# FrozenBurning/SceneDreamer

Hardware: AMD Instinct MI355X
Metric: rendered frames/sec @960×540, 24 samples/ray, scene_size 2048; HBM GB/s (higher is better)
Workload: dtype f16 (3-term split MFMA, f32 accumulate; f32 hash grid); 1 GPU; 960x540, num_samples=24, scene_size=2048, cam pattern 0 (pose stride 2 of 40 poses), 1 frame per rank per step; apron=minimal, parallelism=frames x1

## Files before the change

### scenedreamer_amd/csrc/field.hip

```cpp
#include <hip/hip_fp16.h>

#include <cstdlib>
#include <utility>

#include "field_composite.h"
#include "mlp_layers.h"
#include "sdn_common.h"

namespace {

typedef int i32x4v __attribute__((ext_vector_type(4)));

struct MlpParams {
    const float *feat;
    const float *dist;
    const uint8_t *label;
    const uint8_t *rayflag;
    const half8 *wpk;
    const float *consts;
    const float *sky_c;
    float *net_out;
    int32_t R, ns, nch, n_tiles;
    float term_depth;
    uint8_t *passes;
// ... 109 lines not shown
    const float *u;
    float *rand_depth;
    float *new_dists;
    int64_t *idx;
    int32_t R, M, n_points;
    int32_t ieee_div;
    float sample_depth;
};

__global__ __launch_bounds__(256) void sample_depth_kernel(const SampleParams p) {
    const int ray = blockIdx.x * 256 + threadIdx.x;
    if (ray >= p.R) return;
    RayBoxes rb;
#pragma unroll
    for (int k = 0; k < MAXM; k++) {
        if (k < p.M) {
            rb.t[k] = p.depth2[(size_t)ray * p.M + k];
            rb.t2[k] = p.depth2[((size_t)p.R + ray) * p.M + k];
        } else {
            rb.t[k] = rb.t2[k] = __builtin_nanf("");
        }
        rb.id[k] = 0;
    }
    const float *u = p.u ? p.u + (size_t)ray * p.n_points : nullptr;
    const int ns = p.n_points - 1;
    for (int i = 0; i < ns; i++) {
        Placed pl = place_sample(rb, p.M, p.lin, u, p.ieee_div ? -p.n_points : p.n_points, i, p.sample_depth);
        p.new_dists[(size_t)ray * ns + i] = pl.dist;
        p.rand_depth[(size_t)ray * ns + i] = pl.raw_depth;
        p.idx[(size_t)ray * ns + i] = pl.raw_idx;
    }
}

__device__ __forceinline__ void input_encode(const EncParams &enc, int rr, int rl, int sidx, bool ray_ok, bool use_feat, int h, half8 (&bh)[16],
                                             half8 (&bl)[16], int &lab, float &dist, bool &gnd, float &depth) {
    RayBoxes rb;
    float dd[3];
    enc_load_ray(enc, rr, rb, dd);
    const EncSample es = enc_place(enc, rb, dd, rl, sidx, ray_ok);
    gnd = gnd || es.gnd;
    lab = es.label;
    dist = es.dist;
    depth = es.depth;
#pragma unroll
    for (int b = 0; b < 2; b++) {
        float res[4][8];
        enc_levels<4>(enc, es, 4 * b, h, use_feat, res);
#pragma unroll
        for (int t = 0; t < 4; t++) split8(res[t], bh[4 * b + t], bl[4 * b + t]);
    }
}

template <int DBG>
__device__ __forceinline__ void input_buffer(const MlpParams &p, size_t tc, bool prefetched, bool tile_ok, int lane, int j, half8 (&bh)[16],
                                             half8 (&bl)[16], int &lab, float &dist) {
    float raw[8][8];
    if (prefetched) {
        if constexpr (DBG & 1) asm volatile("s_waitcnt vmcnt(0)" ::: "memory");
        else asm volatile("s_waitcnt vmcnt(16)" ::: "memory");
#define SDN_PF_READ8(S, A0, A1, A2, A3, A4, A5, A6, A7) \
    asm volatile("v_accvgpr_read_b32 %0, a" #A0 "\n\tv_accvgpr_read_b32 %1, a" #A1 "\n\tv_accvgpr_read_b32 %2, a" #A2 \
                 "\n\tv_accvgpr_read_b32 %3, a" #A3 "\n\tv_accvgpr_read_b32 %4, a" #A4 "\n\tv_accvgpr_read_b32 %5, a" #A5 \
                 "\n\tv_accvgpr_read_b32 %6, a" #A6 "\n\tv_accvgpr_read_b32 %7, a" #A7 \
                 : "=v"(raw[S][0]), "=v"(raw[S][1]), "=v"(raw[S][2]), "=v"(raw[S][3]), "=v"(raw[S][4]), "=v"(raw[S][5]), \
                   "=v"(raw[S][6]), "=v"(raw[S][7]))
        SDN_PF_READ8(0, 190, 191, 192, 193, 194, 195, 196, 197);
        SDN_PF_READ8(1, 198, 199, 200, 201, 202, 203, 204, 205);
        SDN_PF_READ8(2, 206, 207, 208, 209, 210, 211, 212, 213);
        SDN_PF_READ8(3, 214, 215, 216, 217, 218, 219, 220, 221);
        SDN_PF_READ8(4, 222, 223, 224, 225, 226, 227, 228, 229);
        SDN_PF_READ8(5, 230, 231, 232, 233, 234, 235, 236, 237);
        SDN_PF_READ8(6, 238, 239, 240, 241, 242, 243, 244, 245);
// ... 41 lines not shown
    asm volatile("global_load_dwordx4 a[" #R0 ":" #R0 "+3], %0, off\n\tglobal_load_dwordx4 a[" #R1 ":" #R1 "+3], %0, off offset:16\n\t" \
                 "global_load_dwordx4 a[" #R2 ":" #R2 "+3], %0, off offset:2048\n\tglobal_load_dwordx4 a[" #R3 ":" #R3 "+3], %0, off offset:2064" \
                 ::"v"(base + (K) * 4096) : "memory", SDN_PF_CLOBBERS)
#define SDN_PF_CLOBBERS "a190", "a191", "a192", "a193", "a194", "a195", "a196", "a197", "a198", "a199", "a200", "a201", "a202", "a203", "a204", "a205", "a206", "a207", "a208", "a209", "a210", "a211", "a212", "a213", "a214", "a215", "a216", "a217", "a218", "a219", "a220", "a221", "a222", "a223", "a224", "a225", "a226", "a227", "a228", "a229", "a230", "a231", "a232", "a233", "a234", "a235", "a236", "a237", "a238", "a239", "a240", "a241", "a242", "a243", "a244", "a245", "a246", "a247", "a248", "a249", "a250", "a251", "a252", "a253"
    SDN_PF_LOAD4(0, 190, 194, 198, 202);
    SDN_PF_LOAD4(1, 206, 210, 214, 218);
    SDN_PF_LOAD4(2, 222, 226, 230, 234);
    SDN_PF_LOAD4(3, 238, 242, 246, 250);
#undef SDN_PF_CLOBBERS
#undef SDN_PF_LOAD4
    asm volatile("global_load_ubyte a254, %0, off" ::"v"(p.label + (size_t)tn * 32 + j) : "memory", "a254");
    asm volatile("global_load_dword a255, %0, off" ::"v"(p.dist + (size_t)tn * 32 + j) : "memory", "a255");
}

__device__ __forceinline__ void flag_put(unsigned flags_a, int word, int v) {
    asm volatile("ds_write_b32 %0, %1" ::"v"(flags_a + 4u * (unsigned)word), "v"(v) : "memory");
}
__device__ __forceinline__ i32x4v flag_get4(unsigned flags_a, int word0) {
    i32x4v f;
    asm volatile("ds_read_b128 %0, %1\n\ts_waitcnt lgkmcnt(0)" : "=v"(f) : "v"(flags_a + 4u * (unsigned)word0) : "memory");
    return f;
}
__device__ __forceinline__ i32x4v workgroup_vote(unsigned flags_a, int word0, int lane, int wave, int mine) {
    if (lane == 0) flag_put(flags_a, word0 + wave, mine);
    asm volatile("s_waitcnt lgkmcnt(0)" ::: "memory");
    __builtin_amdgcn_s_barrier();
    return flag_get4(flags_a, word0);
}

template <int DBG, int CT, int MODE = MODE_BUFFER>
__global__ __launch_bounds__(256, 1) void mlp_kernel(const MlpParams p) {
    constexpr bool FUSED = MODE == MODE_FUSED || MODE == MODE_FUSED_AUX, AUX = MODE == MODE_FUSED_AUX, RAW = MODE == MODE_RAW;
    constexpr bool SKIP = MODE == MODE_FUSED;
    __shared__ __attribute__((aligned(1024))) char lds[LDS_TOTAL];
    const int lane = threadIdx.x & 63, wave = threadIdx.x >> 6;
    const int h = lane >> 5, j = lane & 31;
    const int q = j & 3;

    float *cst = reinterpret_cast<float *>(lds + LDS_CONST);
    stage_consts(cst, p.consts, p.sky_avg);
    EncParams enc = p.enc;
    if constexpr (FUSED)
        stage_enc_tables(enc, p.enc, reinterpret_cast<float *>(lds + LDS_ENC_SCALES), reinterpret_cast<float *>(lds + LDS_ENC_LIN),
                         reinterpret_cast<uint8_t *>(lds + LDS_ENC_LUT), p.cam_ori_dev);
    __syncthreads();

    Ring r;
    r.slots_per_pass = SLOTS_PER_PASS;
    r.wbytes = reinterpret_cast<const char *>(p.wpk);
    r.g = 0;
    r.wave = __builtin_amdgcn_readfirstlane(wave);
    r.lane = lane;
    r.voff = r.wave * (PIECES * 1024) + lane * 16;
    r.lds_lane = (unsigned)(size_t)(const lds_char *)(lds + LDS_RING) + lane * 16;
    r.src_delta = r.wave * (PIECES * 1024) - (int)(unsigned)(size_t)(const lds_char *)(lds + LDS_RING);
#pragma unroll
    for (int sl = 0; sl < DMA_AHEAD; sl++) ring_issue(lds, r, sl, sl);
    r.next_in_pass = DMA_AHEAD;

    unsigned t_seg = 0;
    if constexpr (DBG & 512) {
        if (threadIdx.x < 16) reinterpret_cast<unsigned *>(lds + LDS_TIMERS)[threadIdx.x] = 0u;
        t_seg = (unsigned)__builtin_readcyclecounter();
    }
    long pf_tc = -1;
    unsigned long long t_stage = 0, t_kernel0 = 0;
    unsigned n_pass = 0;
    if constexpr (DBG & 128) t_kernel0 = __builtin_readcyclecounter();
    const int n_groups = (p.n_tiles + 3) >> 2;
    const unsigned flags_a = lds_addr(lds + LDS_FLAGS);
    int grp = blockIdx.x, grp_next = blockIdx.x + (int)gridDim.x;
    auto first_vox = [&](int g) -> int {
        const int t = g * 4 + wave, ry = t * RAYS_PER_TILE + (j >> 2);
        if (!(g < n_groups && t < p.n_tiles && ry < p.R && enc.win.valid(ry))) return 0;
        return enc.voxel_id[(size_t)enc.win.src(ry) * enc.M];
    };
    int vox_cur = 0;
    if constexpr (FUSED) vox_cur = first_vox(grp);
    int cold = 0;
    while (grp < n_groups) {
        const int tile = grp * 4 + wave;
        const bool tile_ok = tile < p.n_tiles;
        const int tile_s = grp * 4 + r.wave;
        const bool tile_ok_s = tile_s < p.n_tiles;
        const int ray = tile * RAYS_PER_TILE + (j >> 2);
        const bool ray_ok = tile_ok && ray < p.R && (!FUSED || p.win.valid(ray));
        const int rl = ray_ok ? ray : p.R - 1;
        const int rr = FUSED ? enc.win.src(rl) : 0;
        uint8_t flag;
        int vox_nxt = 0;
        if constexpr (FUSED) {
            flag = vox_cur != 0 ? (uint8_t)0 : (uint8_t)1;
            vox_nxt = first_vox(grp_next);
        } else if constexpr (RAW) flag = tile_ok ? (uint8_t)0 : (uint8_t)1;
        else flag = ray_ok ? p.rayflag[ray] : (uint8_t)1;
        bool gnd = false;
        int drawn = grp_next + (int)gridDim.x;
        if (p.ticket && threadIdx.x == 0) drawn = 2 * (int)gridDim.x + atomicAdd(p.ticket, 1);
        const bool any_hit = AUX ? tile_ok : __any(!(flag & 1));
        if (threadIdx.x == 0) flag_put(flags_a, 4, drawn);
        const i32x4v fh = workgroup_vote(flags_a, 0, lane, wave, any_hit ? 1 : 0), fd = flag_get4(flags_a, 4);
        const bool grp_hit = __builtin_amdgcn_readfirstlane(fh[0] | fh[1] | fh[2] | fh[3]) != 0;
        const int grp_next2 = __builtin_amdgcn_readfirstlane(fd[0]);
        asm volatile("s_waitcnt lgkmcnt(0)" ::: "memory");
        __builtin_amdgcn_s_barrier();

        float outq[2][4] = {{0.f, 0.f, 0.f, 0.f}, {0.f, 0.f, 0.f, 0.f}};
        float carry = 0.f, tsum = 0.f;
        int n_done = 0, n_colour = 0;
        bool skip_test = SKIP && !p.no_colour_skip && (cold < 6 || (cold & 3) == 0);
        if (SKIP && !skip_test) cold++;

        for (int ch = 0; grp_hit && ch < p.nch; ch++) {
            const size_t tc = (size_t)(tile_ok ? tile : 0) * p.nch + ch;
            half8 bh[16], bl[16];
            f32x16 acc[8];
            MxState mx;
            if constexpr (CT == 6) {
#pragma unroll
                for (int k = 0; k < 4; k++) mx.bm[k] = 0.f;
            }
            seg_tick<DBG>(lds, 9, t_seg);
            unsigned long long t_in0 = 0;
            if constexpr (DBG & 128) t_in0 = __builtin_readcyclecounter();
            const long tc_s = (long)(tile_ok_s ? tile_s : 0) * p.nch + ch;
            int lab;
            float dist;
            float smp_depth = 0.f;
            const long row = (long)(tile_ok ? tile : 0) * 256 + ch * 32 + j;
            if constexpr (RAW) {
                const long rc = row < p.R ? row : (long)p.R - 1;
                lab = p.label[rc];
                dist = 0.f;
                const float *src = p.feat + rc * FEAT + 8 * h;
#pragma unroll
                for (int s = 0; s < 8; s++) {
                    const float4 a = *reinterpret_cast<const float4 *>(src + 16 * s), b = *reinterpret_cast<const float4 *>(src + 16 * s + 4);
                    const float v[8] = {a.x, a.y, a.z, a.w, b.x, b.y, b.z, b.w};
                    split8(v, bh[s], bl[s]);
                }
            }
            else if constexpr (FUSED)
                input_encode(enc, rr, rl, ch * SAMP_PER_STEP + (j & 3), ray_ok, AUX ? ray_ok : !(flag & 1), h, bh, bl, lab, dist, gnd, smp_depth);
            else input_buffer<DBG>(p, tc, pf_tc == tc_s && !(DBG & 256), tile_ok, lane, j, bh, bl, lab, dist);
            if constexpr (DBG & 128) {
                asm volatile("s_waitcnt vmcnt(0)" ::"v"(bh[7]), "v"(bl[7]) : "memory");
                t_stage += __builtin_readcyclecounter() - t_in0;
                n_pass++;
            }
            if constexpr (DBG & 512) asm volatile("s_waitcnt vmcnt(0)" ::"v"(bh[7]), "v"(bl[7]) : "memory");
            seg_tick<DBG>(lds, 0, t_seg);
            float part = 0.f;
            bool colour_skipped = false;
            const float *wsig = cst + C_WSIGMA;
            const float *bias1 = cst + C_LABEL_BIAS + lab * HID;
            layer8<DBG, 8, false, false, false>(lds, r, bh, bl, acc, bias1, bias1, wsig, h, part, TRUNK_K, TRUNK_K);
            act_step<7, false>(acc, bias1, wsig, h, bh, bl, part, TRUNK_K);
            seg_tick<DBG>(lds, 1, t_seg);
#pragma unroll 1
            for (int l = 0; l < 5; l++) {
                const float *bias = cst + C_BETA + l * HID;
                const float *bias_pend = l == 0 ? bias1 : bias - HID;
                constexpr float tk = TRUNK_K;
                if constexpr (CT == 6) {
                    if (l == 2) layer8x<DBG, 0, false, true>(lds, r, bh, bl, mx, acc, bias, bias_pend, wsig, h, part, tk, tk);
                    else if (l == 3) layer8x<DBG, 1, true, false>(lds, r, bh, bl, mx, acc, bias, bias_pend, wsig, h, part, 1.f, tk);
                    else if (l == 4) layer8x<DBG, 2, false, false>(lds, r, bh, bl, mx, acc, bias, bias_pend, wsig, h, part, 1.f, 1.f);
                    else layer8<DBG, 16, true, false, false>(lds, r, bh, bl, acc, bias, bias_pend, wsig, h, part, tk, tk);
                } else {
                    if (l == 2) layer8<DBG, 16, true, false, true, 3, true, CT == 3>(lds, r, bh, bl, acc, bias, bias_pend, wsig, h, part, tk, tk);
                    else if (l == 3) layer8<DBG, 16, true, true, false, CT, CT == 3, CT == 3>(lds, r, bh, bl, acc, bias, bias_pend, wsig, h, part, 1.f, tk);
                    else if (CT != 3 && l == 4) layer8<DBG, 16, true, false, false, CT, CT == 3, true>(lds, r, bh, bl, acc, bias, bias_pend, wsig, h, part, 1.f, 1.f);
                    else if (l == 4) layer8<DBG, 16, true, false, false>(lds, r, bh, bl, acc, bias, bias_pend, wsig, h, part, 1.f, 1.f);
                    else layer8<DBG, 16, true, false, false>(lds, r, bh, bl, acc, bias, bias_pend, wsig, h, part, tk, tk);
                }
                seg_tick<DBG>(lds, 2 + l, t_seg);
                if constexpr (SKIP) {
                    if (l == 2 && skip_test) {
                        float part_e = part;
                        sigma_lower_half(std::make_integer_sequence<int, 16>{}, acc, bias, wsig, h, bh, bl, part_e, tk);
                        const float sigma_e = part_e + __shfl_xor(part_e, 32) + cst[C_BSIGMA];
                        const bool zero_w = !ray_ok || (flag & 1) || fmaxf(sigma_e, 0.f) * dist == 0.f;
                        const int wave_zero = __popcll(__ballot(zero_w));
                        const i32x4v fz = workgroup_vote(flags_a, 8, lane, wave, wave_zero);
                        const int grp_zero = __builtin_amdgcn_readfirstlane(fz[0] + fz[1] + fz[2] + fz[3]);
                        asm volatile("s_waitcnt lgkmcnt(0)" ::: "memory");
                        seg_tick<DBG>(lds, 11, t_seg);
                        skip_test = grp_zero >= 192;
                        if (ch == 0) cold = grp_zero < 64 ? cold + 1 : 0;
                        if (grp_zero == 256) { colour_skipped = true; break; }
                    }
                }
            }
            if constexpr (SKIP) {
                if (colour_skipped) {
                    ring_restart(lds, r);
                    if constexpr (DBG & 512) {
                        if (threadIdx.x == 0) {
                            reinterpret_cast<unsigned *>(lds + LDS_TIMERS)[10] += 1u;
                            reinterpret_cast<unsigned *>(lds + LDS_TIMERS)[12] += 1u;
                        }
                    }
                    n_done = ch + 1;
                    continue;
                }
            }
            n_colour++;
            {
                long tn = tc_s + 1;
                bool has_next = tile_ok_s;
                if (ch + 1 == p.nch) {
                    const int tile2 = grp_next * 4 + r.wave;
                    has_next = tile2 < p.n_tiles;
                    tn = (long)tile2 * p.nch;
                }
                pf_tc = -1;
                if (MODE == MODE_BUFFER && has_next && !(DBG & 256)) {
// ... 9 lines not shown
            const float sigma = part + __shfl_xor(part, 32) + cst[C_BSIGMA];
            if constexpr (RAW) {
                if (tile_ok && row < p.R) {
                    if (h == 0) p.sigma_out[row] = sigma;
                    store_colour_row(p.net_out + (size_t)row * OUTC, col, h);
                }
                n_done = ch + 1;
                continue;
            }
            const float wgt = render_weight(sigma, dist, q, carry);
            tsum += wgt;
            if constexpr (AUX) {
                const int sidx = ch * SAMP_PER_STEP + q;
                if (ray_ok && sidx < p.ns) {
                    const size_t smp = (size_t)p.win.out_row(ray) * p.ns + sidx;
                    if (h == 0) {
                        if (p.w_out) p.w_out[smp] = (flag & 1) ? 0.f : wgt;
                        if (p.depth_out) p.depth_out[smp] = smp_depth;
                        if (p.sig_out) p.sig_out[smp] = sigma;
                    }
                    if (p.col_out) store_colour_row(p.col_out + smp * OUTC, col, h);
                }
            }
            accumulate_colour(col, wgt, q, outq);
            if constexpr (DBG & 512) {
                asm volatile("" ::"v"(outq[0][0]), "v"(outq[1][3]), "v"(carry), "v"(tsum));
                seg_tick<DBG>(lds, 8, t_seg);
                if (threadIdx.x == 0) reinterpret_cast<unsigned *>(lds + LDS_TIMERS)[10] += 1u;
            }
            n_done = ch + 1;
            if (p.term_depth > 0.f && ch + 1 < p.nch) {
                const bool opaque = !ray_ok || (flag & 1) || carry > p.term_depth;
                const bool wave_done = __all(opaque);
                const i32x4v ft = workgroup_vote(flags_a, 0, lane, wave, wave_done ? 1 : 0);
                const bool grp_done = __builtin_amdgcn_readfirstlane(ft[0] & ft[1] & ft[2] & ft[3]) != 0;
                asm volatile("s_waitcnt lgkmcnt(0)" ::: "memory");
                __builtin_amdgcn_s_barrier();
                if (grp_done) break;
            }
        }
#ifndef SDN_NO_TERM_GND
        if constexpr (FUSED) {
            if (grp_hit && n_done < p.nch) {
                RayBoxes rb;
                float dd[3];
                enc_load_ray(enc, rr, rb, dd);
#pragma unroll 1
                for (int c2 = n_done; c2 < p.nch; c2++)
                    gnd = gnd || enc_place(enc, rb, dd, rl, c2 * SAMP_PER_STEP + (j & 3), ray_ok).gnd;
            }
        }
#endif
        if (p.passes && threadIdx.x == 0) p.passes[grp] = (uint8_t)n_done;
        if (p.colour_passes && threadIdx.x == 0) p.colour_passes[grp] = (uint8_t)n_colour;

        if constexpr (!RAW) {
            if constexpr (FUSED) {
                const int g = quad_any(gnd);
                const bool last_hit = ray_ok && enc.voxel_id[(size_t)rr * enc.M + (enc.M - 1)] != 0;
                if (last_hit || g) flag |= 2;
            }
            blend_sky_store<AUX>(cst, p.sky_c, p.net_out, p.win.src(ray), p.win.out_row(ray), ray_ok, tsum, flag, outq, q, h,
                                 p.skyb_out, p.nosky_out);
        }
        grp = grp_next;
        grp_next = grp_next2;
        vox_cur = vox_nxt;
    }
    asm volatile("s_waitcnt vmcnt(0)" ::: "memory");
    __builtin_amdgcn_s_barrier();
    if (p.ticket && threadIdx.x == 0 && atomicAdd(p.ticket + 1, 1) == (int)gridDim.x - 1) {
        p.ticket[0] = 0;
        p.ticket[1] = 0;
    }
    if constexpr (DBG & 512) {
        __syncthreads();
        if (threadIdx.x < 13) p.net_out[(size_t)(blockIdx.x * 4) * OUTC + 3 + threadIdx.x] = (float)reinterpret_cast<unsigned *>(lds + LDS_TIMERS)[threadIdx.x];
    }
    if constexpr (DBG & 128) {
        if (lane == 0) {
            float *o = p.net_out + (size_t)(blockIdx.x * 4 + wave) * OUTC;
            o[0] = (float)t_stage; o[1] = (float)(__builtin_readcyclecounter() - t_kernel0); o[2] = (float)n_pass;
        }
    }
}

__global__ void mfma_probe_kernel(const float *A, const float *B, float *C) {
    const int lane = threadIdx.x, h = lane >> 5, j = lane & 31;
    half8 a, b;
#pragma unroll
    for (int e = 0; e < 8; e++) {
        a[e] = (_Float16)A[j * 16 + 8 * h + e];
        b[e] = (_Float16)B[(8 * h + e) * 32 + j];
    }
    f32x16 c;
#pragma unroll
    for (int r = 0; r < 16; r++) c[r] = 0.f;
    c = mfma16(a, b, c);
#pragma unroll
    for (int r = 0; r < 16; r++) C[((r & 3) + 8 * (r >> 2) + 4 * h) * 32 + j] = c[r];
// ... 247 lines not shown
```

### scenedreamer_amd/csrc/field_enc.h

```cpp
#pragma once
#include "mlp_layers.h"
#include "sdn_common.h"

namespace {

constexpr int RAYS_PER_TILE = 8;
constexpr int SAMP_PER_STEP = 4;
constexpr int MAXM = 8;

struct RayWindow {
    int32_t n_src;
    int32_t pitch, first, cols, ray0;
    int32_t tiled_bx;
    int32_t rows;
    __device__ __forceinline__ int pix(int r) const {
        const int w = ray0 + r;
        if (tiled_bx == 0) return w;
        const int b = w >> 5, by = b / tiled_bx, bxi = b - by * tiled_bx;
        const int y = 4 * by + ((w & 31) >> 3), x = 8 * bxi + (w & 7);
        if (rows > 0 && (x >= cols || y >= rows)) return -1;
        return y * cols + x;
    }
    __device__ __forceinline__ bool valid(int r) const { return rows == 0 || pix(r) >= 0; }
    __device__ __forceinline__ int src(int r) const {
// ... 16 lines not shown
    uint8_t *label;
    uint8_t *rayflag;
    int32_t R, M, ns, nch, n_tiles;
    uint32_t tmask;
    float ori[3], delim[3];
    float sample_depth, dists_scale;
    int32_t genc_oob;
    int32_t ieee_div;
    const float *lin;
    const float *u;
    const float *scales;
    RayWindow win;
};

struct RayBoxes {
    float t[MAXM], t2[MAXM];
    int32_t id[MAXM];
};

struct Placed {
    float depth, dist;
    int idx;
    float raw_depth;
    int raw_idx;
};

__device__ __forceinline__ float strat_pos(const float *lin, const float *u, int n_div, int i) {
#pragma clang fp contract(off)
    if (u == nullptr) return lin[i];
    const float q = n_div > 0 ? u[i] * (1.0f / (float)n_div) : u[i] / (float)(-n_div);
    return q + lin[i];
}

__device__ __forceinline__ Placed place_sample(const RayBoxes &rb, int M, const float *lin, const float *u, int n_div, int sidx,
                                               float sample_depth) {
#pragma clang fp contract(off)
    float accu[MAXM];
    double run_d = 0.0;
    float run = 0.f;
#pragma unroll
    for (int k = 0; k < MAXM; k++) {
        if (k < M) {
            float d = rb.t2[k] - rb.t[k];
            if (d != d) d = 0.f;
            run_d += (double)d;
            run = (float)run_d;
            accu[k] = run;
        } else {
            accu[k] = 0.f;
        }
    }
    const float total = fminf(run, sample_depth);
    const float s0 = strat_pos(lin, u, n_div, sidx) * total, s1 = strat_pos(lin, u, n_div, sidx + 1) * total;
    const float mid = (s1 + s0) / 2.f;
    Placed o;
    o.dist = s1 - s0;
    int idx = 0;
#pragma unroll
    for (int k = 0; k < MAXM; k++)
        if (k < M && mid > accu[k]) idx++;
    float head = rb.t[0];
    double cg_d = 0.0;
#pragma unroll
    for (int k = 1; k < MAXM; k++) {
        if (k < M) {
            const float g = rb.t[k] - rb.t2[k - 1];
            cg_d += (double)g;
            const float cg = (float)cg_d;
            if (k == idx) head = cg + rb.t[0];
        }
    }
    float depth = head + mid;
    o.raw_depth = depth;
    o.raw_idx = idx;
    if (depth != depth || __builtin_isinf(depth)) depth = 0.f;
    o.depth = depth;
    o.idx = idx < M ? idx : M - 1;
    return o;
}

__device__ __forceinline__ float mul_add_exact(float a, float b, float c) {
#pragma clang fp contract(off)
    const float p = a * b;
    return p + c;
}

__device__ __forceinline__ float normalise_coord(float wc, float delim) {
#pragma clang fp contract(off)
    float n = wc / delim;
    n = n * 2.f;
    n = n - 1.f;
    n = n + 1.f;
    return n / 2.f;
}

__device__ __forceinline__ void enc_load_ray(const EncParams &p, int rr, RayBoxes &rb, float (&d)[3]) {
    const size_t RS = (size_t)p.win.n_src;
#pragma unroll
    for (int k = 0; k < MAXM; k++) {
        if (k < p.M) {
            rb.t[k] = p.depth2[(size_t)rr * p.M + k];
            rb.t2[k] = p.depth2[(RS + rr) * p.M + k];
            rb.id[k] = p.voxel_id[(size_t)rr * p.M + k];
        } else {
            rb.t[k] = rb.t2[k] = __builtin_nanf("");
            rb.id[k] = 0;
        }
    }
    d[0] = p.raydirs[(size_t)rr * 3]; d[1] = p.raydirs[(size_t)rr * 3 + 1]; d[2] = p.raydirs[(size_t)rr * 3 + 2];
}

struct EncSample {
    float x0, x1, x2;
    bool oob, valid, gnd;
    float dist;
    int label;
    float depth;
};

__device__ __forceinline__ EncSample enc_place(const EncParams &p, const RayBoxes &rb, const float (&d)[3], int rl, int sidx, bool ray_ok) {
    EncSample e;
    e.valid = ray_ok && sidx < p.ns;
    const Placed pl = place_sample(rb, p.M, p.lin, p.u ? p.u + (size_t)p.win.out_row(rl) * (p.ns + 1) : nullptr, p.ieee_div ? -(p.ns + 1) : p.ns + 1,
                                   e.valid ? sidx : 0, p.sample_depth);
    const float wx = mul_add_exact(d[0], pl.depth, p.ori[0]);
    const float wy = mul_add_exact(d[1], pl.depth, p.ori[1]);
    const float wz = mul_add_exact(d[2], pl.depth, p.ori[2]);
    e.gnd = e.valid && wx <= 1.0f;
    e.x0 = normalise_coord(wx, p.delim[0]);
    e.x1 = normalise_coord(wy, p.delim[1]);
    e.x2 = normalise_coord(wz, p.delim[2]);
    e.oob = p.genc_oob || e.x0 < 0.f || e.x0 > 1.f || e.x1 < 0.f || e.x1 > 1.f || e.x2 < 0.f || e.x2 > 1.f;
    e.dist = e.valid ? pl.dist * p.dists_scale : 0.f;
    e.depth = pl.depth;
    int id = rb.id[0];
#pragma unroll
    for (int k = 1; k < MAXM; k++) {
        id = k == pl.idx ? rb.id[k] : id;
        asm("" : "+v"(id));
    }
    e.label = p.lut[id & 1023];
    return e;
}

struct LevelAddr {
    float f0, f1, f2;
    uint32_t off[8];
};

__device__ __forceinline__ void enc_level_addr(const EncParams &p, const EncSample &e, int level, bool ok, LevelAddr &a) {
    const float scale = p.scales[level];
    float f0 = mul_add_exact(e.x0, scale, 0.5f), f1 = mul_add_exact(e.x1, scale, 0.5f), f2 = mul_add_exact(e.x2, scale, 0.5f);
    const float g0 = floorf(f0), g1 = floorf(f1), g2 = floorf(f2);
    a.f0 = f0 - g0; a.f1 = f1 - g1; a.f2 = f2 - g2;
    const uint32_t a0 = (uint32_t)g0, a1 = (uint32_t)g1 * 2654435761u, a2 = (uint32_t)g2 * 805459861u;
    const uint32_t b0 = a0 + 1u, b1 = a1 + 2654435761u, b2 = a2 + 805459861u;
    const uint32_t tb = (uint32_t)level * (p.tmask + 1u);
#pragma unroll
    for (int c = 0; c < 8; c++) {
        const uint32_t hsh = ((c & 1) ? b0 : a0) ^ ((c & 2) ? b1 : a1) ^ ((c & 4) ? b2 : a2);
        a.off[c] = (tb + (ok ? (hsh & p.tmask) : 0u)) * 32u;
    }
}

__device__ __forceinline__ void enc_level_load(const EncParams &p, const LevelAddr &a, float4 (&va)[8], float4 (&vb)[8]) {
    const char *base = reinterpret_cast<const char *>(p.table3);
#pragma unroll
    for (int c = 0; c < 8; c++) {
        va[c] = *reinterpret_cast<const float4 *>(base + a.off[c]);
        vb[c] = *reinterpret_cast<const float4 *>(base + a.off[c] + 16);
    }
}

__device__ __forceinline__ void enc_level_blend(const LevelAddr &a, const float4 (&va)[8], const float4 (&vb)[8], float (&res)[8]) {
    float2v r01 = {0.f, 0.f}, r23 = {0.f, 0.f}, r45 = {0.f, 0.f}, r67 = {0.f, 0.f};
// ... 113 lines not shown
```

### scenedreamer_amd/csrc/mlp_layers.h

```cpp
#pragma once

#include <utility>

#include "mfma_common.h"

namespace {

constexpr int HID = 256;
constexpr int FEAT = 128;
constexpr int OUTC = 64;
constexpr int NLEV = 16;
constexpr int NLAB = 12;
constexpr int MAX_LIN = 80;
constexpr float ACT_SCALE = 0.4f;
#ifndef SDN_TRUNK_SHIFT
#define SDN_TRUNK_SHIFT 8
#endif
constexpr int TRUNK_SHIFT = SDN_TRUNK_SHIFT;
constexpr float TRUNK_K = 1.0f / (float)(1 << TRUNK_SHIFT);

constexpr size_t L0_FRAGS = 8 * 8 * 2 * 64;
constexpr size_t LH_FRAGS = 16 * 8 * 2 * 64;
constexpr size_t LO_FRAGS = 16 * 2 * 2 * 64;
constexpr size_t PACKED_FRAGS = L0_FRAGS + 5 * LH_FRAGS + LO_FRAGS;
// ... 23 lines not shown
constexpr int QUAD_LAST = 0xFF;
constexpr int DPP_ROW_HALF_MIRROR = 0x141;
constexpr int DPP_ROW_MIRROR = 0x140;

__device__ __forceinline__ void split8(const float (&v)[8], half8 &hi, half8 &lo) {
    unsigned int hw[4], lw[4];
#pragma unroll
    for (int e = 0; e < 8; e += 2) {
        const half2v hp = cvt_rtn(v[e], v[e + 1]);
        const half2v lp = cvt_rtn(v[e] - (float)hp[0], v[e + 1] - (float)hp[1]);
        hw[e / 2] = __builtin_bit_cast(unsigned int, hp);
        lw[e / 2] = __builtin_bit_cast(unsigned int, lp);
    }
    typedef unsigned int u32x4 __attribute__((ext_vector_type(4)));
    u32x4 h4 = {hw[0], hw[1], hw[2], hw[3]}, l4 = {lw[0], lw[1], lw[2], lw[3]};
    hi = __builtin_bit_cast(half8, h4);
    lo = __builtin_bit_cast(half8, l4);
}

constexpr int UNITS_PER_SLOT = 8;
constexpr int NSLOT = 4;
constexpr int SLOT_BYTES = UNITS_PER_SLOT * 4096;
constexpr int DMA_AHEAD = 3;
constexpr int PIECES = SLOT_BYTES / 4096;
constexpr int SLOTS_PER_PASS = (8 + 5 * 16 + 4) * 4 / UNITS_PER_SLOT;
constexpr int LDS_RING = 0;
constexpr int LDS_CONST = NSLOT * SLOT_BYTES;
constexpr int LDS_FLAGS = LDS_CONST + ((C_TOTAL * 4 + 255) / 256) * 256;
constexpr int LDS_ENC_SCALES = LDS_FLAGS + 64;
constexpr int LDS_ENC_LIN = LDS_ENC_SCALES + NLEV * 4;
constexpr int LDS_ENC_LUT = LDS_ENC_LIN + MAX_LIN * 4;
constexpr int LDS_TIMERS = LDS_ENC_LUT + 1024;
constexpr int LDS_TOTAL = LDS_TIMERS + 64;

__device__ __forceinline__ f32x16 zero16() {
    f32x16 z;
#pragma unroll
    for (int r = 0; r < 16; r++) z[r] = 0.f;
    return z;
}

__device__ __forceinline__ void store_colour_row(float *dst, const f32x16 (&col)[2], int h) {
#pragma unroll
    for (int ib = 0; ib < 2; ib++)
#pragma unroll
        for (int g4 = 0; g4 < 4; g4++)
            *reinterpret_cast<float4 *>(dst + 32 * ib + 8 * g4 + 4 * h) =
                make_float4(col[ib][4 * g4], col[ib][4 * g4 + 1], col[ib][4 * g4 + 2], col[ib][4 * g4 + 3]);
}

struct Ring {
    int slots_per_pass;
    const char *wbytes;
    int g;
    int next_in_pass;
    int wave;
    int lane;
    int voff;
    unsigned lds_lane;
    int src_delta;
    int pend_global, pend_in_pass;
    const char *pend_src;
};

__device__ __forceinline__ const char *ring_lane_src(const char *slot_base, const Ring &r) {
    unsigned int lo, hi;
// ... 648 lines not shown
```

### scenedreamer_amd/fused.py

```python
import ctypes
import math
import os

import numpy as np
import torch

from . import capi
from .precision import TERM_EPS_DEFAULT
from .timing import _time_ms

_f2 = ctypes.c_float * 2
_f3 = ctypes.c_float * 3
_i6 = ctypes.c_int32 * 6


AUX_OUTPUTS = ("weights", "depth", "sigma", "colour", "sky_blended", "nosky")


class Window:

    def __init__(self, n_src, pitch=0, first=0, rows=None, cols=0):
        self.n_src, self.pitch, self.first, self.cols = int(n_src), int(pitch), int(first), int(cols)
        self.rows = rows
        self.n_rays = int(rows * cols) if cols else int(n_src)
# ... 289 lines not shown
    ct, eps = precision_profile(R)
    assert sky_c.is_contiguous() and sky_avg.is_contiguous() and sky_avg.numel() == 64 and sky_avg.dtype == torch.float32
    if not (sky_c.is_cuda and sky_avg.is_cuda and sky_c.device == R.dev == sky_avg.device and net_out.device == R.dev):
        raise ValueError(f"sky_c / sky_avg / net_out must live on {R.dev} (got {sky_c.device}, {sky_avg.device}, {net_out.device})")
    if window is None:
        window = Window(sky_c.shape[0])
    if "ticket" not in st:
        st["ticket"] = torch.zeros(2, dtype=torch.int32, device=R.dev)
    with torch.cuda.device(R.dev):
        rc = _lib().sdn_field_mlp(buf["feat"].data_ptr(), buf["dist"].data_ptr(), buf["label"].data_ptr(),
                                  buf["rayflag"].data_ptr(), st["packed_mx" if ct == 6 else "packed"].data_ptr(),
                                  st["consts"].data_ptr(), sky_c.data_ptr(), net_out.data_ptr(), n_rays, ns, ct, eps,
                                  passes.data_ptr() if passes is not None else None, 0, window.host(ray0, n_rays),
                                  sky_avg.data_ptr(), st["ticket"].data_ptr() if dynamic else None, _stream(R.dev))
    capi.check(rc, "sdn_field_mlp")


def mlp_from(R, buf, sky_c, sky_avg, n_rays, ns, window=None):
    st = R._fused_style or prepare_style(R)
    net_out = torch.empty((n_rays, 64), dtype=torch.float32, device=R.dev)
    _launch_mlp(R, buf, st, sky_c, sky_avg, net_out, n_rays, ns, window=window)
    return net_out


def single_kernel(R):
    return R.resolved_single_kernel()


def colour_skip(R):
    return R.resolved_colour_skip()


def field_render(R, vid, d2, rd, cam_ori, sky_c, sky_avg, ns, passes=None, u=None, window=None, division="reciprocal",
                 net_out=None, aux=None, colour_passes=None):
    sc = R._fused_scene or prepare_scene(R)
    st = R._fused_style or prepare_style(R)
    ct, eps = precision_profile(R)
    if aux is not None:
        eps = 0.0
    if ct == 2:
        raise ValueError("the single-kernel field supports colour_terms 3 and 6")
    if window is None:
        window = Window(vid.shape[0])
    n_rays = window.n_rays

    def addr(t, rows, what):
        if isinstance(t, int):
            return t
        assert t.is_cuda and t.device == R.dev and t.is_contiguous() and t.shape[rows] == window.n_src, what
        return t.data_ptr()

    if not isinstance(sky_c, int):
        sky_c = sky_c.contiguous()
    p_vid, p_d2, p_rd, p_sky = addr(vid, 0, "voxel_id"), addr(d2, 1, "depth2"), addr(rd, 0, "raydirs"), addr(sky_c, 0, "sky_c")
    sky_avg = _sky_avg(R, sky_avg)
    if net_out is None:
        net_out = torch.empty((n_rays, 64), dtype=torch.float32, device=R.dev)
    if u is not None:
        assert u.is_cuda and u.dtype == torch.float32 and tuple(u.shape) == (n_rays, ns + 1) and u.is_contiguous()
    lin = _lin(R, ns, stratified=u is not None)
    if "ticket" not in st:
        st["ticket"] = torch.zeros(2, dtype=torch.int32, device=R.dev)
    ori, ori_dev = _cam_ori(R, cam_ori)
    aux_c = None
    if aux is not None:
        aux_c = _aux_tensors(R, aux, n_rays, ns)
    ragged = u is None and all(t is None or t.numel() >= window.n_groups(ragged=True) for t in (passes, colour_passes))
    skip = colour_skip(R)
    if colour_passes is not None or not skip:
        aux_c = aux_c or capi.FieldAux()
        aux_c.colour_passes = colour_passes.data_ptr() if colour_passes is not None else None
        aux_c.flags = 0 if skip else capi.FIELD_NO_COLOUR_SKIP
    with torch.cuda.device(R.dev):
        rc = _lib().sdn_field_render(p_vid, p_d2, p_rd, sc["lut"].data_ptr(), sc["table3"].data_ptr(),
                                     sc["T"], sc["scales"].data_ptr(), sc["genc"].ctypes.data, ori.ctypes.data,
                                     sc["dims"].ctypes.data, lin.data_ptr(), u.data_ptr() if u is not None else None, n_rays, R.M,
                                     ns, R.sample_depth, R.dists_scale, st["packed_mx" if ct == 6 else "packed"].data_ptr(),
                                     st["consts"].data_ptr(), p_sky, sky_avg.data_ptr(), net_out.data_ptr(), ct, eps,
                                     passes.data_ptr() if passes is not None else None, 0, window.host(0, n_rays, ragged),
                                     {"reciprocal": 0, "ieee": 1}[division], st["ticket"].data_ptr(),
                                     ori_dev.data_ptr() if ori_dev is not None else None,
                                     ctypes.byref(aux_c) if aux_c is not None else None, _stream(R.dev))
    capi.check(rc, "sdn_field_render")
    return net_out


def _per_ray_feat_bytes(ns):
    return _lib().sdn_field_feat_bytes(32, ns) // 32


def single_chunk(n_rays, ns):
    return n_rays * _per_ray_feat_bytes(ns) <= FEATURE_BUFFER_BYTES


def field_fused(R, vid, d2, rd, cam_ori, sky_c, sky_avg, ns, passes=None, u=None, window=None, division="reciprocal"):
    st = R._fused_style or prepare_style(R)
    if window is None:
        window = Window(vid.shape[0])
    n_rays = window.n_rays
    vid, d2, rd, sky_c = vid.contiguous(), d2.contiguous(), rd.contiguous(), sky_c.contiguous()
    if single_kernel(R) and precision_profile(R)[0] != 2:
        return field_render(R, vid, d2, rd, cam_ori, sky_c, sky_avg, ns, passes=passes, u=u, window=window, division=division)
    sky_avg = torch.as_tensor(sky_avg).reshape(-1).to(device=R.dev, dtype=torch.float32).contiguous()
    net_out = torch.empty((n_rays, 64), dtype=torch.float32, device=R.dev)
    chunk = max(32, (FEATURE_BUFFER_BYTES // _per_ray_feat_bytes(ns)) // 32 * 32)
    for r0 in range(0, n_rays, chunk):
        n = min(n_rays, r0 + chunk) - r0
        uc = u[r0:r0 + n].contiguous() if u is not None else None
        buf = encode(R, vid, d2, rd, cam_ori, ns, u=uc, window=window, ray0=r0, n_rays=n, division=division)
        _launch_mlp(R, buf, st, sky_c, sky_avg, net_out[r0:r0 + n], n, ns, passes[r0 // 32:] if passes is not None else None,
                    window=window, ray0=r0)
    return net_out
# ... 112 lines not shown
```

Baseline: 56.56 frames/s.

## Prefetch per-ray box rows into LDS and cache per-ray placement state

In the fused field kernel, each wave now asynchronously copies the next group's depth, voxel-id and ray-direction rows into LDS with global_load_lds while the current group is processed. One lane per ray then computes the per-ray cumulative box lengths and heads once and stores them in an LDS RayState slot. Every sample placement reads that cached state instead of reloading the rows from global memory and redoing the double-precision prefix sums. This replaces repeated global loads and per-sample prefix work with LDS reads. In exchange the kernel uses more LDS, adds inline-asm waitcnt handling, and adds an n_workgroups parameter to the Python launcher.

```diff
diff --git a/scenedreamer_amd/csrc/field.hip b/scenedreamer_amd/csrc/field.hip
--- a/scenedreamer_amd/csrc/field.hip
+++ b/scenedreamer_amd/csrc/field.hip
@@ -165,12 +165,112 @@
     }
 }
 
-__device__ __forceinline__ void input_encode(const EncParams &enc, int rr, int rl, int sidx, bool ray_ok, bool use_feat, int h, half8 (&bh)[16],
-                                             half8 (&bl)[16], int &lab, float &dist, bool &gnd, float &depth) {
-    RayBoxes rb;
+
+template <int STRIDE>
+__device__ __forceinline__ unsigned ray_slot_addr(unsigned wave_base) {
+    unsigned a;
+    asm volatile("v_mbcnt_lo_u32_b32 %0, -1, 0\n\t"
+                 "v_mbcnt_hi_u32_b32 %0, -1, %0\n\t"
+                 "v_bfe_u32 %0, %0, 2, 3\n\t"
+                 "v_mul_u32_u24 %0, %2, %0\n\t"
+                 "v_add_u32 %0, %1, %0"
+                 : "=&v"(a)
+                 : "s"(wave_base), "n"(STRIDE));
+    return a;
+}
+
+__device__ __forceinline__ void group_rows_fetch(const EncParams &enc, char *graw_wave, int wave_s, int g, int n_groups) {
+    int lane;
+    asm volatile("v_mbcnt_lo_u32_b32 %0, -1, 0\n\tv_mbcnt_hi_u32_b32 %0, -1, %0" : "=&v"(lane));
+    const int t = g * 4 + wave_s, ry = t * RAYS_PER_TILE + (lane >> 3);
+    const bool ok = g < n_groups && t < enc.n_tiles && ry < enc.R && enc.win.valid(ry);
+    const size_t rr = (size_t)enc.win.src(ok ? ry : enc.R - 1), RS = (size_t)enc.win.n_src;
+    const int k = lane & 7, kb = k < enc.M ? k : enc.M - 1, kd = k < 3 ? k : 2;
+    const char *t_src = reinterpret_cast<const char *>(enc.depth2 + rr * enc.M + kb);
+    const char *t2_src = reinterpret_cast<const char *>(enc.depth2 + (RS + rr) * enc.M + kb);
+    const char *id_src = reinterpret_cast<const char *>(enc.voxel_id + rr * enc.M + kb);
+    const char *d_src = reinterpret_cast<const char *>(enc.raydirs + rr * 3 + kd);
+    __builtin_amdgcn_global_load_lds((glb_char *)t_src, (lds_char *)graw_wave, 4, 0, 0);
+    __builtin_amdgcn_global_load_lds((glb_char *)t2_src, (lds_char *)(graw_wave + 256), 4, 0, 0);
+    __builtin_amdgcn_global_load_lds((glb_char *)id_src, (lds_char *)(graw_wave + 512), 4, 0, 0);
+    __builtin_amdgcn_global_load_lds((glb_char *)d_src, (lds_char *)(graw_wave + 768), 4, 0, 0);
+}
+
+__device__ __forceinline__ void graw_read(unsigned a, int M, RayBoxes &rb, float (&d)[3]) {
+    f32x4 t0, t1, u0, u1, dv;
+    i32x4v i0, i1;
+    asm volatile("ds_read_b128 %0, %7\n\t"
+                 "ds_read_b128 %1, %7 offset:16\n\t"
+                 "ds_read_b128 %2, %7 offset:256\n\t"
+                 "ds_read_b128 %3, %7 offset:272\n\t"
+                 "ds_read_b128 %4, %7 offset:512\n\t"
+                 "ds_read_b128 %5, %7 offset:528\n\t"
+                 "ds_read_b128 %6, %7 offset:768\n\t"
+                 "s_waitcnt lgkmcnt(0)"
+                 : "=&v"(t0), "=&v"(t1), "=&v"(u0), "=&v"(u1), "=&v"(i0), "=&v"(i1), "=&v"(dv)
+                 : "v"(a)
+                 : "memory");
+#pragma unroll
+    for (int k = 0; k < MAXM; k++) {
+        const bool in = k < M;
+        rb.t[k] = in ? (k < 4 ? t0[k & 3] : t1[k & 3]) : __builtin_nanf("");
+        rb.t2[k] = in ? (k < 4 ? u0[k & 3] : u1[k & 3]) : __builtin_nanf("");
+        rb.id[k] = in ? (k < 4 ? i0[k & 3] : i1[k & 3]) : 0;
+    }
+    d[0] = dv[0]; d[1] = dv[1]; d[2] = dv[2];
+}
+
+__device__ __forceinline__ void gstate_write(unsigned a, const RayState &st, const float (&d)[3]) {
+    const f32x4 a0 = {st.accu[0], st.accu[1], st.accu[2], st.accu[3]}, a1 = {st.accu[4], st.accu[5], st.accu[6], st.accu[7]};
+    const f32x4 h0 = {st.head[0], st.head[1], st.head[2], st.head[3]}, h1 = {st.head[4], st.head[5], st.head[6], st.head[7]};
+    const i32x4v i0 = {st.id[0], st.id[1], st.id[2], st.id[3]}, i1 = {st.id[4], st.id[5], st.id[6], st.id[7]};
+    const f32x4 td = {st.total, d[0], d[1], d[2]};
+    asm volatile("ds_write_b128 %0, %1\n\t"
+                 "ds_write_b128 %0, %2 offset:16\n\t"
+                 "ds_write_b128 %0, %3 offset:32\n\t"
+                 "ds_write_b128 %0, %4 offset:48\n\t"
+                 "ds_write_b128 %0, %5 offset:64\n\t"
+                 "ds_write_b128 %0, %6 offset:80\n\t"
+                 "ds_write_b128 %0, %7 offset:96\n\t"
+                 "s_waitcnt lgkmcnt(0)"
+                 :: "v"(a), "v"(a0), "v"(a1), "v"(h0), "v"(h1), "v"(i0), "v"(i1), "v"(td)
+                 : "memory");
+}
+__device__ __forceinline__ void gstate_read(unsigned a, RayState &st, float (&d)[3]) {
+    f32x4 a0, a1, h0, h1, td;
+    i32x4v i0, i1;
+    asm volatile("ds_read_b128 %0, %7\n\t"
+                 "ds_read_b128 %1, %7 offset:16\n\t"
+                 "ds_read_b128 %2, %7 offset:32\n\t"
+                 "ds_read_b128 %3, %7 offset:48\n\t"
+                 "ds_read_b128 %4, %7 offset:64\n\t"
+                 "ds_read_b128 %5, %7 offset:80\n\t"
+                 "ds_read_b128 %6, %7 offset:96\n\t"
+                 "s_waitcnt lgkmcnt(0)"
+                 : "=&v"(a0), "=&v"(a1), "=&v"(h0), "=&v"(h1), "=&v"(i0), "=&v"(i1), "=&v"(td)
+                 : "v"(a)
+                 : "memory");
+#pragma unroll
+    for (int k = 0; k < MAXM; k++) {
+        st.accu[k] = k < 4 ? a0[k & 3] : a1[k & 3];
+        st.head[k] = k < 4 ? h0[k & 3] : h1[k & 3];
+        st.id[k] = k < 4 ? i0[k & 3] : i1[k & 3];
+    }
+    st.total = td[0];
+    d[0] = td[1]; d[1] = td[2]; d[2] = td[3];
+}
+__device__ __forceinline__ int gstate_read_id(unsigned a, int k) {
+    int v;
+    asm volatile("ds_read_b32 %0, %1 offset:64\n\ts_waitcnt lgkmcnt(0)" : "=v"(v) : "v"(a + 4u * (unsigned)k) : "memory");
+    return v;
+}
+
+__device__ __forceinline__ void input_encode(const EncParams &enc, unsigned gstate_wave_a, int rl, int sidx, bool ray_ok, bool use_feat, int h,
+                                             half8 (&bh)[16], half8 (&bl)[16], int &lab, float &dist, bool &gnd, float &depth) {
+    RayState st;
     float dd[3];
-    enc_load_ray(enc, rr, rb, dd);
-    const EncSample es = enc_place(enc, rb, dd, rl, sidx, ray_ok);
+    gstate_read(ray_slot_addr<GSTATE_RAY_BYTES>(gstate_wave_a), st, dd);
+    const EncSample es = enc_place(enc, st, dd, rl, sidx, ray_ok);
     gnd = gnd || es.gnd;
     lab = es.label;
     dist = es.dist;
@@ -278,7 +378,7 @@
 __global__ __launch_bounds__(256, 1) void mlp_kernel(const MlpParams p) {
     constexpr bool FUSED = MODE == MODE_FUSED || MODE == MODE_FUSED_AUX, AUX = MODE == MODE_FUSED_AUX, RAW = MODE == MODE_RAW;
     constexpr bool SKIP = MODE == MODE_FUSED;
-    __shared__ __attribute__((aligned(1024))) char lds[LDS_TOTAL];
+    __shared__ __attribute__((aligned(1024))) char lds[FUSED ? LDS_TOTAL_FIELD : LDS_TOTAL];
     const int lane = threadIdx.x & 63, wave = threadIdx.x >> 6;
     const int h = lane >> 5, j = lane & 31;
     const int q = j & 3;
@@ -316,28 +416,30 @@
     const int n_groups = (p.n_tiles + 3) >> 2;
     const unsigned flags_a = lds_addr(lds + LDS_FLAGS);
     int grp = blockIdx.x, grp_next = blockIdx.x + (int)gridDim.x;
-    auto first_vox = [&](int g) -> int {
-        const int t = g * 4 + wave, ry = t * RAYS_PER_TILE + (j >> 2);
-        if (!(g < n_groups && t < p.n_tiles && ry < p.R && enc.win.valid(ry))) return 0;
-        return enc.voxel_id[(size_t)enc.win.src(ry) * enc.M];
-    };
-    int vox_cur = 0;
-    if constexpr (FUSED) vox_cur = first_vox(grp);
+    char *const graw_wave = lds + LDS_GRAW + r.wave * GRAW_WAVE_BYTES;
+    const unsigned graw_wave_a = lds_addr(lds + LDS_GRAW) + (unsigned)(r.wave * GRAW_WAVE_BYTES);
+    const unsigned gstate_wave_a = lds_addr(lds + LDS_GSTATE) + (unsigned)(r.wave * RAYS_PER_TILE * GSTATE_RAY_BYTES);
+    if constexpr (FUSED) {
+        group_rows_fetch(enc, graw_wave, r.wave, grp, n_groups);
+        asm volatile("s_waitcnt vmcnt(0)" ::: "memory");
+    }
     int cold = 0;
     while (grp < n_groups) {
-        const int tile = grp * 4 + wave;
+        const int wave_g = FUSED ? r.wave : wave;
+        const int tile = grp * 4 + wave_g;
         const bool tile_ok = tile < p.n_tiles;
         const int tile_s = grp * 4 + r.wave;
         const bool tile_ok_s = tile_s < p.n_tiles;
         const int ray = tile * RAYS_PER_TILE + (j >> 2);
         const bool ray_ok = tile_ok && ray < p.R && (!FUSED || p.win.valid(ray));
-        const int rl = ray_ok ? ray : p.R - 1;
-        const int rr = FUSED ? enc.win.src(rl) : 0;
         uint8_t flag;
-        int vox_nxt = 0;
         if constexpr (FUSED) {
-            flag = vox_cur != 0 ? (uint8_t)0 : (uint8_t)1;
-            vox_nxt = first_vox(grp_next);
+            RayBoxes rb;
+            float dd[3];
+            graw_read(ray_slot_addr<32>(graw_wave_a), enc.M, rb, dd);
+            group_rows_fetch(enc, graw_wave, r.wave, grp_next, n_groups);
+            if ((lane & 35) == 0) gstate_write(ray_slot_addr<GSTATE_RAY_BYTES>(gstate_wave_a), place_ray(rb, enc.M, enc.sample_depth), dd);
+            flag = ray_ok && rb.id[0] != 0 ? (uint8_t)0 : (uint8_t)1;
         } else if constexpr (RAW) flag = tile_ok ? (uint8_t)0 : (uint8_t)1;
         else flag = ray_ok ? p.rayflag[ray] : (uint8_t)1;
         bool gnd = false;
@@ -345,7 +447,7 @@
         if (p.ticket && threadIdx.x == 0) drawn = 2 * (int)gridDim.x + atomicAdd(p.ticket, 1);
         const bool any_hit = AUX ? tile_ok : __any(!(flag & 1));
         if (threadIdx.x == 0) flag_put(flags_a, 4, drawn);
-        const i32x4v fh = workgroup_vote(flags_a, 0, lane, wave, any_hit ? 1 : 0), fd = flag_get4(flags_a, 4);
+        const i32x4v fh = workgroup_vote(flags_a, 0, lane, wave_g, any_hit ? 1 : 0), fd = flag_get4(flags_a, 4);
         const bool grp_hit = __builtin_amdgcn_readfirstlane(fh[0] | fh[1] | fh[2] | fh[3]) != 0;
         const int grp_next2 = __builtin_amdgcn_readfirstlane(fd[0]);
         asm volatile("s_waitcnt lgkmcnt(0)" ::: "memory");
@@ -387,7 +489,7 @@
                 }
             }
             else if constexpr (FUSED)
-                input_encode(enc, rr, rl, ch * SAMP_PER_STEP + (j & 3), ray_ok, AUX ? ray_ok : !(flag & 1), h, bh, bl, lab, dist, gnd, smp_depth);
+                input_encode(enc, gstate_wave_a, ray_ok ? ray : p.R - 1, ch * SAMP_PER_STEP + (j & 3), ray_ok, AUX ? ray_ok : !(flag & 1), h, bh, bl, lab, dist, gnd, smp_depth);
             else input_buffer<DBG>(p, tc, pf_tc == tc_s && !(DBG & 256), tile_ok, lane, j, bh, bl, lab, dist);
             if constexpr (DBG & 128) {
                 asm volatile("s_waitcnt vmcnt(0)" ::"v"(bh[7]), "v"(bl[7]) : "memory");
@@ -428,7 +530,7 @@
                         const float sigma_e = part_e + __shfl_xor(part_e, 32) + cst[C_BSIGMA];
                         const bool zero_w = !ray_ok || (flag & 1) || fmaxf(sigma_e, 0.f) * dist == 0.f;
                         const int wave_zero = __popcll(__ballot(zero_w));
-                        const i32x4v fz = workgroup_vote(flags_a, 8, lane, wave, wave_zero);
+                        const i32x4v fz = workgroup_vote(flags_a, 8, lane, wave_g, wave_zero);
                         const int grp_zero = __builtin_amdgcn_readfirstlane(fz[0] + fz[1] + fz[2] + fz[3]);
                         asm volatile("s_waitcnt lgkmcnt(0)" ::: "memory");
                         seg_tick<DBG>(lds, 11, t_seg);
@@ -504,7 +606,7 @@
             if (p.term_depth > 0.f && ch + 1 < p.nch) {
                 const bool opaque = !ray_ok || (flag & 1) || carry > p.term_depth;
                 const bool wave_done = __all(opaque);
-                const i32x4v ft = workgroup_vote(flags_a, 0, lane, wave, wave_done ? 1 : 0);
+                const i32x4v ft = workgroup_vote(flags_a, 0, lane, wave_g, wave_done ? 1 : 0);
                 const bool grp_done = __builtin_amdgcn_readfirstlane(ft[0] & ft[1] & ft[2] & ft[3]) != 0;
                 asm volatile("s_waitcnt lgkmcnt(0)" ::: "memory");
                 __builtin_amdgcn_s_barrier();
@@ -514,12 +616,12 @@
 #ifndef SDN_NO_TERM_GND
         if constexpr (FUSED) {
             if (grp_hit && n_done < p.nch) {
-                RayBoxes rb;
+                RayState st;
                 float dd[3];
-                enc_load_ray(enc, rr, rb, dd);
+                gstate_read(ray_slot_addr<GSTATE_RAY_BYTES>(gstate_wave_a), st, dd);
 #pragma unroll 1
                 for (int c2 = n_done; c2 < p.nch; c2++)
-                    gnd = gnd || enc_place(enc, rb, dd, rl, c2 * SAMP_PER_STEP + (j & 3), ray_ok).gnd;
+                    gnd = gnd || enc_place(enc, st, dd, ray_ok ? ray : p.R - 1, c2 * SAMP_PER_STEP + (j & 3), ray_ok).gnd;
             }
         }
 #endif
@@ -529,15 +631,18 @@
         if constexpr (!RAW) {
             if constexpr (FUSED) {
                 const int g = quad_any(gnd);
-                const bool last_hit = ray_ok && enc.voxel_id[(size_t)rr * enc.M + (enc.M - 1)] != 0;
+                const int last_id = gstate_read_id(ray_slot_addr<GSTATE_RAY_BYTES>(gstate_wave_a), enc.M - 1);
+                const bool last_hit = ray_ok && last_id != 0;
                 if (last_hit || g) flag |= 2;
             }
             blend_sky_store<AUX>(cst, p.sky_c, p.net_out, p.win.src(ray), p.win.out_row(ray), ray_ok, tsum, flag, outq, q, h,
                                  p.skyb_out, p.nosky_out);
         }
+        if constexpr (FUSED) {
+            if (!grp_hit) asm volatile("s_waitcnt vmcnt(0)" ::: "memory");
+        }
         grp = grp_next;
         grp_next = grp_next2;
-        vox_cur = vox_nxt;
     }
     asm volatile("s_waitcnt vmcnt(0)" ::: "memory");
     __builtin_amdgcn_s_barrier();
diff --git a/scenedreamer_amd/csrc/field_enc.h b/scenedreamer_amd/csrc/field_enc.h
--- a/scenedreamer_amd/csrc/field_enc.h
+++ b/scenedreamer_amd/csrc/field_enc.h
@@ -72,10 +72,16 @@
     return q + lin[i];
 }
 
-__device__ __forceinline__ Placed place_sample(const RayBoxes &rb, int M, const float *lin, const float *u, int n_div, int sidx,
-                                               float sample_depth) {
-#pragma clang fp contract(off)
+struct RayState {
     float accu[MAXM];
+    float head[MAXM];
+    int32_t id[MAXM];
+    float total;
+};
+
+__device__ __forceinline__ RayState place_ray(const RayBoxes &rb, int M, float sample_depth) {
+#pragma clang fp contract(off)
+    RayState st;
     double run_d = 0.0;
     float run = 0.f;
 #pragma unroll
@@ -85,12 +91,31 @@
             if (d != d) d = 0.f;
             run_d += (double)d;
             run = (float)run_d;
-            accu[k] = run;
+            st.accu[k] = run;
         } else {
-            accu[k] = 0.f;
+            st.accu[k] = 0.f;
         }
-    }
-    const float total = fminf(run, sample_depth);
+        st.id[k] = rb.id[k];
+    }
+    st.total = fminf(run, sample_depth);
+    st.head[0] = rb.t[0];
+    double cg_d = 0.0;
+#pragma unroll
+    for (int k = 1; k < MAXM; k++) {
+        st.head[k] = rb.t[0];
+        if (k < M) {
+            const float g = rb.t[k] - rb.t2[k - 1];
+            cg_d += (double)g;
+            const float cg = (float)cg_d;
+            st.head[k] = cg + rb.t[0];
+        }
+    }
+    return st;
+}
+
+__device__ __forceinline__ Placed place_in_ray(const RayState &st, int M, const float *lin, const float *u, int n_div, int sidx) {
+#pragma clang fp contract(off)
+    const float total = st.total;
     const float s0 = strat_pos(lin, u, n_div, sidx) * total, s1 = strat_pos(lin, u, n_div, sidx + 1) * total;
     const float mid = (s1 + s0) / 2.f;
     Placed o;
@@ -98,17 +123,12 @@
     int idx = 0;
 #pragma unroll
     for (int k = 0; k < MAXM; k++)
-        if (k < M && mid > accu[k]) idx++;
-    float head = rb.t[0];
-    double cg_d = 0.0;
+        if (k < M && mid > st.accu[k]) idx++;
+    float head = st.head[0];
 #pragma unroll
     for (int k = 1; k < MAXM; k++) {
-        if (k < M) {
-            const float g = rb.t[k] - rb.t2[k - 1];
-            cg_d += (double)g;
-            const float cg = (float)cg_d;
-            if (k == idx) head = cg + rb.t[0];
-        }
+        head = (k < M && k == idx) ? st.head[k] : head;
+        asm("" : "+v"(head));
     }
     float depth = head + mid;
     o.raw_depth = depth;
@@ -117,6 +137,11 @@
     o.depth = depth;
     o.idx = idx < M ? idx : M - 1;
     return o;
+}
+
+__device__ __forceinline__ Placed place_sample(const RayBoxes &rb, int M, const float *lin, const float *u, int n_div, int sidx,
+                                               float sample_depth) {
+    return place_in_ray(place_ray(rb, M, sample_depth), M, lin, u, n_div, sidx);
 }
 
 __device__ __forceinline__ float mul_add_exact(float a, float b, float c) {
@@ -158,11 +183,11 @@
     float depth;
 };
 
-__device__ __forceinline__ EncSample enc_place(const EncParams &p, const RayBoxes &rb, const float (&d)[3], int rl, int sidx, bool ray_ok) {
+__device__ __forceinline__ EncSample enc_place(const EncParams &p, const RayState &st, const float (&d)[3], int rl, int sidx, bool ray_ok) {
     EncSample e;
     e.valid = ray_ok && sidx < p.ns;
-    const Placed pl = place_sample(rb, p.M, p.lin, p.u ? p.u + (size_t)p.win.out_row(rl) * (p.ns + 1) : nullptr, p.ieee_div ? -(p.ns + 1) : p.ns + 1,
-                                   e.valid ? sidx : 0, p.sample_depth);
+    const Placed pl = place_in_ray(st, p.M, p.lin, p.u ? p.u + (size_t)p.win.out_row(rl) * (p.ns + 1) : nullptr, p.ieee_div ? -(p.ns + 1) : p.ns + 1,
+                                   e.valid ? sidx : 0);
     const float wx = mul_add_exact(d[0], pl.depth, p.ori[0]);
     const float wy = mul_add_exact(d[1], pl.depth, p.ori[1]);
     const float wz = mul_add_exact(d[2], pl.depth, p.ori[2]);
@@ -173,14 +198,18 @@
     e.oob = p.genc_oob || e.x0 < 0.f || e.x0 > 1.f || e.x1 < 0.f || e.x1 > 1.f || e.x2 < 0.f || e.x2 > 1.f;
     e.dist = e.valid ? pl.dist * p.dists_scale : 0.f;
     e.depth = pl.depth;
-    int id = rb.id[0];
+    int id = st.id[0];
 #pragma unroll
     for (int k = 1; k < MAXM; k++) {
-        id = k == pl.idx ? rb.id[k] : id;
+        id = k == pl.idx ? st.id[k] : id;
         asm("" : "+v"(id));
     }
     e.label = p.lut[id & 1023];
     return e;
+}
+
+__device__ __forceinline__ EncSample enc_place(const EncParams &p, const RayBoxes &rb, const float (&d)[3], int rl, int sidx, bool ray_ok) {
+    return enc_place(p, place_ray(rb, p.M, p.sample_depth), d, rl, sidx, ray_ok);
 }
 
 struct LevelAddr {
diff --git a/scenedreamer_amd/csrc/mlp_layers.h b/scenedreamer_amd/csrc/mlp_layers.h
--- a/scenedreamer_amd/csrc/mlp_layers.h
+++ b/scenedreamer_amd/csrc/mlp_layers.h
@@ -79,6 +79,13 @@
 constexpr int LDS_ENC_LUT = LDS_ENC_LIN + MAX_LIN * 4;
 constexpr int LDS_TIMERS = LDS_ENC_LUT + 1024;
 constexpr int LDS_TOTAL = LDS_TIMERS + 64;
+constexpr int GSTATE_RAY_BYTES = 112;
+constexpr int GRAW_WAVE_BYTES = 1024;
+constexpr int LDS_GSTATE = LDS_TOTAL;
+constexpr int LDS_GRAW = LDS_GSTATE + 32 * GSTATE_RAY_BYTES;
+constexpr int LDS_TOTAL_FIELD = LDS_GRAW + 4 * GRAW_WAVE_BYTES;
+static_assert(LDS_GSTATE % 16 == 0 && GSTATE_RAY_BYTES % 16 == 0 && LDS_GRAW % 16 == 0, "ds_read_b128 / ds_write_b128 need 16-byte alignment");
+static_assert(LDS_TOTAL_FIELD <= 160 * 1024, "the field kernel's LDS must fit the CU's 160 KiB");
 
 __device__ __forceinline__ f32x16 zero16() {
     f32x16 z;
diff --git a/scenedreamer_amd/fused.py b/scenedreamer_amd/fused.py
--- a/scenedreamer_amd/fused.py
+++ b/scenedreamer_amd/fused.py
@@ -345,7 +345,7 @@
 
 
 def field_render(R, vid, d2, rd, cam_ori, sky_c, sky_avg, ns, passes=None, u=None, window=None, division="reciprocal",
-                 net_out=None, aux=None, colour_passes=None):
+                 net_out=None, aux=None, colour_passes=None, n_workgroups=0):
     sc = R._fused_scene or prepare_scene(R)
     st = R._fused_style or prepare_style(R)
     ct, eps = precision_profile(R)
@@ -390,7 +390,7 @@
                                      sc["dims"].ctypes.data, lin.data_ptr(), u.data_ptr() if u is not None else None, n_rays, R.M,
                                      ns, R.sample_depth, R.dists_scale, st["packed_mx" if ct == 6 else "packed"].data_ptr(),
                                      st["consts"].data_ptr(), p_sky, sky_avg.data_ptr(), net_out.data_ptr(), ct, eps,
-                                     passes.data_ptr() if passes is not None else None, 0, window.host(0, n_rays, ragged),
+                                     passes.data_ptr() if passes is not None else None, int(n_workgroups), window.host(0, n_rays, ragged),
                                      {"reciprocal": 0, "ieee": 1}[division], st["ticket"].data_ptr(),
                                      ori_dev.data_ptr() if ori_dev is not None else None,
                                      ctypes.byref(aux_c) if aux_c is not None else None, _stream(R.dev))
```

After: 56.49 frames/s. No clear change (-0.1%).
